# mjq11302010044/TATT

Hardware: AMD Instinct MI355X
Metric: LR images/s (train fwd+bwd+clip+Adam) at 16x64->32x128 (higher is better)
Workload: dtype fp32 (split-bf16 MFMA operands in conv3 / conv3-wgrad / conv9 / tokgemm / gru-wgrad / query-GRU recurrence and dW_hh / TP-layer backward)

## Files before the change

### tatt_amd/csrc/conv9.hip

```cpp
#include "common.h"
#include <mutex>

#define T9_H 8
#define T9_W 32
#define T9_HH (T9_H + 8)
#define T9_WW (T9_W + 8)
#define T9_CK 16

__device__ __forceinline__ void stage_halo_q(const float* __restrict__ x, f32x4 (*Xs)[T9_HH][T9_WW], int n, int h0, int w0,
                                             int H, int W, int C, int c0) {
    for (int i = threadIdx.x; i < T9_HH * T9_WW * 4; i += 256) {
        const int c4 = i & 3, p = i >> 2;
        const int r = p / T9_WW, cc = p - r * T9_WW;
        const int hh = h0 + r - 4, ww = w0 + cc - 4;
        f32x4 v = (f32x4){0.f, 0.f, 0.f, 0.f};
        if (hh >= 0 && hh < H && ww >= 0 && ww < W)
            v = *reinterpret_cast<const f32x4*>(x + (((long)n * H + hh) * W + ww) * C + c0 + 4 * c4);
        Xs[c4][r][cc] = v;
    }
}

__global__ __launch_bounds__(256) void conv9_c64_to_c4_kernel(const float* __restrict__ x, const float* __restrict__ wp,
                                                              const float* __restrict__ bias, float* __restrict__ y,
                                                              int B, int H, int W, int C) {
    __shared__ f32x4 Xs[4][T9_HH][T9_WW];
    const int tiles_w = W / T9_W, tiles_h = H / T9_H;
    int bid = blockIdx.x;
    const int tw = bid % tiles_w; bid /= tiles_w;
    const int th = bid % tiles_h; const int n = bid / tiles_h;
    const int h0 = th * T9_H, w0 = tw * T9_W;
    const int tx = threadIdx.x & 31, ty = threadIdx.x >> 5;
    float a0 = 0.f, a1 = 0.f, a2 = 0.f, a3 = 0.f;
    for (int c0 = 0; c0 < C; c0 += T9_CK) {
        __syncthreads();
        stage_halo_q(x, Xs, n, h0, w0, H, W, C, c0);
        __syncthreads();
        for (int kh = 0; kh < 9; ++kh) {
#pragma unroll
            for (int kw = 0; kw < 9; ++kw) {
                const float* wt = wp + ((long)(kh * 9 + kw) * C + c0) * 4;
#pragma unroll
                for (int c4 = 0; c4 < 4; ++c4) {
                    const f32x4 v = Xs[c4][ty + kh][tx + kw];
#pragma unroll
                    for (int u = 0; u < 4; ++u) {
                        const float* wv = wt + (c4 * 4 + u) * 4;
                        a0 = fmaf(v[u], wv[0], a0); a1 = fmaf(v[u], wv[1], a1);
                        a2 = fmaf(v[u], wv[2], a2); a3 = fmaf(v[u], wv[3], a3);
                    }
                }
            }
        }
    }
    if (bias) { a0 += bias[0]; a1 += bias[1]; a2 += bias[2]; a3 += bias[3]; }
    const long o = (((long)n * H + h0 + ty) * W + w0 + tx) * 4;
    *reinterpret_cast<f32x4*>(y + o) = (f32x4){a0, a1, a2, a3};
}
TATT_API int tatt_conv9_c64_to_c4(const float* x, const float* wpacked, const float* bias, float* y, int B, int H, int W,
                                  int C, hipStream_t st) {
    if (C % T9_CK || H % T9_H || W % T9_W) return 1;
    hipLaunchKernelGGL(conv9_c64_to_c4_kernel, dim3(B * (H / T9_H) * (W / T9_W)), dim3(256), 0, st, x, wpacked, bias, y, B,
                       H, W, C);
    return LAUNCH_CHECK();
}

#define M9_TH 4
#define M9_TW 64
#define M9_PW 96
#define M9_ROWS (M9_TH + 8)
#define M9_HPX (M9_ROWS * 72)
#define M9_HQ 2
#define M9_D 3
#define M9_XS (M9_ROWS * 16 * M9_PW)
__global__ __launch_bounds__(512) void conv9_c64_to_c4_mfma_kernel(const float* __restrict__ x, const float* __restrict__ wt,
                                                                   const float* __restrict__ bias, float* __restrict__ y,
                                                                   int B, int H, int W, int ntiles) {
    __shared__ __attribute__((aligned(16))) float Xs[M9_XS];
    __shared__ __attribute__((aligned(16))) float Red[4 * 64 * 4];
    const int t = threadIdx.x, lane = t & 63, wave = t >> 6;
    const int row = wave & 3, kh = wave >> 2;
    const int tiles_w = W / M9_TW, tiles_h = H / M9_TH;
    const int i = lane & 15, kq = lane >> 4;
    const int g = (i & 8) ? i : (i ^ 4);
    const float* xa = Xs + (row * 16 + 4 * kh + kq) * M9_PW + 4 * g;
    const int wl = (kh * 6 * 64 + lane) * 16;
    const __amdgpu_buffer_rsrc_t wrs = __builtin_amdgcn_make_buffer_rsrc(const_cast<float*>(wt), 0, 9 * 4 * 2 * 6 * 64 * 4 * 4, 0x00020000);
    f32x4 wpre[M9_D + 1][6];
    f32x4 hpre[M9_HQ][4];
    auto filt_load = [&](int p) {
#pragma unroll
        for (int f = 0; f < 6; ++f)
            wpre[p % (M9_D + 1)][f] = __builtin_bit_cast(f32x4, __builtin_amdgcn_raw_buffer_load_b128(
                wrs, wl, (((p % 9) * 4 + p / 9) * 12 + f) * 1024, 0));
    };
    auto halo_load = [&](int tile, int c0, int q) {
        const int tw = tile % tiles_w, th = (tile / tiles_w) % tiles_h, n = tile / (tiles_w * tiles_h);
        const int pp = t + 512 * q;
        const int r = pp / 72, px = pp - r * 72;
        const int hh = th * M9_TH + r - 4, ww = tw * M9_TW + px - 4;
        const bool ok = tile < ntiles && pp < M9_HPX && hh >= 0 && hh < H && ww >= 0 && ww < W;
        const f32x4* src = reinterpret_cast<const f32x4*>(x + (((long)n * H + hh) * W + ww) * 64 + c0);
#pragma unroll
        for (int c4 = 0; c4 < 4; ++c4) hpre[q][c4] = ok ? src[c4] : (f32x4){0.f, 0.f, 0.f, 0.f};
    };
    auto halo_store = [&](int q) {
        const int pp = t + 512 * q;
        if (pp < M9_HPX) {
            const int r = pp / 72, px = pp - r * 72;
            float* d = Xs + r * 16 * M9_PW + px;
#pragma unroll
            for (int c4 = 0; c4 < 4; ++c4)
#pragma unroll
                for (int e = 0; e < 4; ++e) d[(4 * c4 + e) * M9_PW] = hpre[q][c4][e];
        }
    };
#pragma unroll
    for (int q = 0; q < M9_D; ++q) filt_load(q);
#pragma unroll
    for (int q = 0; q < M9_HQ; ++q) halo_load(blockIdx.x, 0, q);
#pragma unroll
    for (int q = 0; q < M9_HQ; ++q) halo_store(q);
    __syncthreads();
    const float bo = bias ? bias[i & 3] : 0.f;
#pragma unroll 1
    for (int tile = blockIdx.x; tile < ntiles; tile += gridDim.x) {
        f32x4 acc4[4];
#pragma unroll
        for (int q = 0; q < 4; ++q) acc4[q] = (f32x4){0.f, 0.f, 0.f, 0.f};
#pragma unroll
        for (int c = 0; c < 4; ++c) {
#pragma unroll
            for (int ky = 0; ky < 9; ++ky) {
                const int p = 9 * c + ky;
                filt_load((p + M9_D) % 36);
                if (ky < M9_HQ) {
                    if (c < 3) halo_load(tile, 16 * (c + 1), ky);
                    else halo_load(tile + gridDim.x, 0, ky);
                }
#pragma unroll
                for (int d = 0; d < 3; ++d) {
                    const f32x4 a0 = *reinterpret_cast<const f32x4*>(xa + (ky * 16 + 0) * M9_PW + 4 * d);
                    const f32x4 a1 = *reinterpret_cast<const f32x4*>(xa + (ky * 16 + 8) * M9_PW + 4 * d);
                    const f32x4 b0 = wpre[p % (M9_D + 1)][d], b1 = wpre[p % (M9_D + 1)][3 + d];
#pragma unroll
                    for (int u = 0; u < 4; ++u) {
                        acc4[u & 1] = __builtin_amdgcn_mfma_f32_16x16x4f32(a0[u], b0[u], acc4[u & 1], 0, 0, 0);
                        acc4[2 + (u & 1)] = __builtin_amdgcn_mfma_f32_16x16x4f32(a1[u], b1[u], acc4[2 + (u & 1)], 0, 0, 0);
                    }
                }
                __builtin_amdgcn_sched_barrier(0);
                if (ky == 8) {
                    f32x4 acc = (acc4[0] + acc4[1]) + (acc4[2] + acc4[3]);
                    __syncthreads();
#pragma unroll
                    for (int q = 0; q < M9_HQ; ++q) halo_store(q);
                    if (c == 3 && kh == 1) *reinterpret_cast<f32x4*>(&Red[(row * 64 + lane) * 4]) = acc;
                    __syncthreads();
                    if (c == 3 && kh == 0) {
                        acc += *reinterpret_cast<const f32x4*>(&Red[(row * 64 + lane) * 4]);
                        const int tw = tile % tiles_w, th = (tile / tiles_w) % tiles_h, n = tile / (tiles_w * tiles_h);
#pragma unroll
                        for (int reg = 0; reg < 4; ++reg) {
                            const int mrow = 4 * kq + reg;
                            const int gg = (mrow & 8) ? mrow : (mrow ^ 4);
                            y[(((long)n * H + th * M9_TH + row) * W + tw * M9_TW + 4 * gg) * 4 + i] = acc[reg] + bo;
                        }
                    }
                }
            }
        }
    }
}
TATT_API int tatt_conv9_c64_to_c4_mfma(const float* x, const float* wt, const float* bias, float* y, int B, int H, int W,
                                       hipStream_t st) {
    if (H % M9_TH || W % M9_TW) return 1;
    const int ntiles = B * (H / M9_TH) * (W / M9_TW);
    hipLaunchKernelGGL(conv9_c64_to_c4_mfma_kernel, dim3(ntiles < 256 ? ntiles : 256), dim3(512), 0, st, x, wt, bias, y, B, H, W,
                       ntiles);
    return LAUNCH_CHECK();
}

#define S9_ROWB (4 * 18 * 32)
#define S9_IMG (M9_ROWS * S9_ROWB)
#define S9_THREADS 768
#define S9_D 5
#define S9_RED (12 * 2 * 64 * 16)
#define S9_LDS (2 * S9_IMG + S9_RED)
typedef __bf16 s9_bf16x8 __attribute__((ext_vector_type(8)));
typedef __bf16 s9_bf16x2 __attribute__((ext_vector_type(2)));
typedef float s9_f32x2 __attribute__((ext_vector_type(2)));
typedef unsigned s9_u32x4 __attribute__((ext_vector_type(4)));
__device__ __forceinline__ void s9_split(f32x4 v, unsigned& h0, unsigned& h1, unsigned& l0, unsigned& l1) {
    const s9_f32x2 a = (s9_f32x2){v[0], v[1]}, b = (s9_f32x2){v[2], v[3]};
    const s9_bf16x2 ha = __builtin_convertvector(a, s9_bf16x2), hb = __builtin_convertvector(b, s9_bf16x2);
    const s9_bf16x2 la = __builtin_convertvector(a - __builtin_convertvector(ha, s9_f32x2), s9_bf16x2);
    const s9_bf16x2 lb = __builtin_convertvector(b - __builtin_convertvector(hb, s9_f32x2), s9_bf16x2);
    h0 = __builtin_bit_cast(unsigned, ha); h1 = __builtin_bit_cast(unsigned, hb);
    l0 = __builtin_bit_cast(unsigned, la); l1 = __builtin_bit_cast(unsigned, lb);
}
__global__ __launch_bounds__(S9_THREADS) void conv9_c64_to_c4_sb_kernel(const float* __restrict__ x, const float* __restrict__ wt,
                                                                        const float* __restrict__ bias, float* __restrict__ y,
                                                                        int B, int H, int W, int ntiles) {
    extern __shared__ __attribute__((aligned(16))) unsigned char s9_lds[];
    unsigned char* const Xs = s9_lds;
    float* const Red = reinterpret_cast<float*>(s9_lds + 2 * S9_IMG);
    const int t = threadIdx.x, lane = t & 63;
    const int wave = __builtin_amdgcn_readfirstlane(t >> 6);
    const int pair = wave % 6, rh = wave / 6;
    const int tiles_w = W / M9_TW, tiles_h = H / M9_TH;
    const int i = lane & 15, kq = lane >> 4;
    const int pair_off = (((2 * pair) & 3) * 18 + (pair >> 1)) * 32;
    int xa[2];
#pragma unroll
    for (int r = 0; r < 2; ++r) xa[r] = (((2 * rh + r) * 4 + (kq >> 1)) * 18 + i) * 32 + (kq & 1) * 16 + pair_off;
    const int wl = (pair * 2 * 64 + lane) * 16;
    const __amdgpu_buffer_rsrc_t wrs = __builtin_amdgcn_make_buffer_rsrc(const_cast<float*>(wt), 0, 9 * 4 * 2 * 6 * 64 * 4 * 4, 0x00020000);
    f32x4 wpre[S9_D + 1][2];
    f32x4 hpre[M9_HQ][4];
    auto filt_load = [&](int p) {
#pragma unroll
        for (int f = 0; f < 2; ++f)
            wpre[p % (S9_D + 1)][f] = __builtin_bit_cast(f32x4, __builtin_amdgcn_raw_buffer_load_b128(
                wrs, wl, (((p % 9) * 4 + p / 9) * 12 + f) * 1024, 0));
    };
    auto halo_load = [&](int tile, int c0, int q) {
        const int tw = tile % tiles_w, th = (tile / tiles_w) % tiles_h, n = tile / (tiles_w * tiles_h);
        const int pp = t + S9_THREADS * q;
        const int r = pp / 72, px = pp - r * 72;
        const int hh = th * M9_TH + r - 4, ww = tw * M9_TW + px - 4;
        const bool ok = tile < ntiles && pp < M9_HPX && hh >= 0 && hh < H && ww >= 0 && ww < W;
        const f32x4* src = reinterpret_cast<const f32x4*>(x + (((long)n * H + hh) * W + ww) * 64 + c0);
#pragma unroll
        for (int c4 = 0; c4 < 4; ++c4) hpre[q][c4] = ok ? src[c4] : (f32x4){0.f, 0.f, 0.f, 0.f};
    };
    auto halo_store = [&](int q) {
        const int pp = t + S9_THREADS * q;
        if (pp < M9_HPX) {
            const int r = pp / 72, px = pp - r * 72;
            unsigned char* d = Xs + ((r * 4 + (px & 3)) * 18 + (px >> 2)) * 32;
            unsigned h[8], l[8];
#pragma unroll
            for (int c4 = 0; c4 < 4; ++c4) s9_split(hpre[q][c4], h[2 * c4], h[2 * c4 + 1], l[2 * c4], l[2 * c4 + 1]);
            *reinterpret_cast<s9_u32x4*>(d) = (s9_u32x4){h[0], h[1], h[2], h[3]};
            *reinterpret_cast<s9_u32x4*>(d + 16) = (s9_u32x4){h[4], h[5], h[6], h[7]};
            *reinterpret_cast<s9_u32x4*>(d + S9_IMG) = (s9_u32x4){l[0], l[1], l[2], l[3]};
            *reinterpret_cast<s9_u32x4*>(d + S9_IMG + 16) = (s9_u32x4){l[4], l[5], l[6], l[7]};
        }
    };
    const int per_img = tiles_w * tiles_h;
    const bool by_xcd = (gridDim.x & 7) == 0 && (B & 7) == 0;
    const int xcd = blockIdx.x & 7, wg_m = blockIdx.x >> 3, wg_M = gridDim.x >> 3;
    auto tile_of = [&](int s) -> int {
        if (!by_xcd) { const long tl = (long)blockIdx.x + (long)s * gridDim.x; return tl < ntiles ? (int)tl : ntiles; }
        const int sq = wg_m + s * wg_M, img = xcd + 8 * (sq / per_img);
        return img < B ? img * per_img + sq % per_img : ntiles;
    };
#pragma unroll
    for (int q = 0; q < S9_D; ++q) filt_load(q);
#pragma unroll
    for (int q = 0; q < M9_HQ; ++q) halo_load(tile_of(0), 0, q);
#pragma unroll
    for (int q = 0; q < M9_HQ; ++q) halo_store(q);
    __syncthreads();
    const float bo = bias ? bias[i & 3] : 0.f;
#pragma unroll 1
    for (int ts = 0;; ++ts) {
        const int tile = tile_of(ts);
        if (tile >= ntiles) break;
        const int tile_next = tile_of(ts + 1);
        f32x4 acc6[2][3];
#pragma unroll
        for (int q = 0; q < 6; ++q) acc6[q / 3][q % 3] = (f32x4){0.f, 0.f, 0.f, 0.f};
#pragma unroll
        for (int c = 0; c < 4; ++c) {
#pragma unroll
            for (int ky = 0; ky < 9; ++ky) {
                const int p = 9 * c + ky;
                filt_load((p + S9_D) % 36);
                if (ky < M9_HQ) {
                    if (c < 3) halo_load(tile, 16 * (c + 1), ky);
                    else halo_load(tile_next, 0, ky);
                }
                const s9_bf16x8 bh = __builtin_bit_cast(s9_bf16x8, wpre[p % (S9_D + 1)][0]);
                const s9_bf16x8 bl = __builtin_bit_cast(s9_bf16x8, wpre[p % (S9_D + 1)][1]);
                s9_bf16x8 ah[2], al[2];
#pragma unroll
                for (int r = 0; r < 2; ++r) {
                    ah[r] = *reinterpret_cast<const s9_bf16x8*>(Xs + xa[r] + ky * S9_ROWB);
                    al[r] = *reinterpret_cast<const s9_bf16x8*>(Xs + xa[r] + ky * S9_ROWB + S9_IMG);
                }
#pragma unroll
                for (int r = 0; r < 2; ++r) {
                    acc6[r][0] = __builtin_amdgcn_mfma_f32_16x16x32_bf16(ah[r], bh, acc6[r][0], 0, 0, 0);
                    acc6[r][1] = __builtin_amdgcn_mfma_f32_16x16x32_bf16(ah[r], bl, acc6[r][1], 0, 0, 0);
                    acc6[r][2] = __builtin_amdgcn_mfma_f32_16x16x32_bf16(al[r], bh, acc6[r][2], 0, 0, 0);
                }
                __builtin_amdgcn_sched_barrier(0);
                if (ky == 8) {
                    __syncthreads();
#pragma unroll
                    for (int q = 0; q < M9_HQ; ++q) halo_store(q);
                    if (c == 3) {
#pragma unroll
                        for (int r = 0; r < 2; ++r)
                            *reinterpret_cast<f32x4*>(&Red[((wave * 2 + r) * 64 + lane) * 4]) = (acc6[r][0] + acc6[r][1]) + acc6[r][2];
                    }
                    __syncthreads();
                    if (c == 3 && pair < 2) {
                        f32x4 acc = (f32x4){0.f, 0.f, 0.f, 0.f};
#pragma unroll
                        for (int pw = 0; pw < 6; ++pw)
                            acc += *reinterpret_cast<const f32x4*>(&Red[(((rh * 6 + pw) * 2 + pair) * 64 + lane) * 4]);
                        const int tw = tile % tiles_w, th = (tile / tiles_w) % tiles_h, n = tile / (tiles_w * tiles_h);
#pragma unroll
                        for (int reg = 0; reg < 4; ++reg)
                            y[(((long)n * H + th * M9_TH + 2 * rh + pair) * W + tw * M9_TW + 4 * (4 * kq + reg)) * 4 + i] = acc[reg] + bo;
                    }
                }
            }
        }
    }
}
TATT_API int tatt_conv9_c64_to_c4_sb(const float* x, const float* wt, const float* bias, float* y, int B, int H, int W,
                                     hipStream_t st) {
    if (H % M9_TH || W % M9_TW) return 1;
    const int ntiles = B * (H / M9_TH) * (W / M9_TW);
    static TattPerDevice attr_once;
    tatt_per_device(attr_once, [&] {
        (void)hipFuncSetAttribute(reinterpret_cast<const void*>(conv9_c64_to_c4_sb_kernel), hipFuncAttributeMaxDynamicSharedMemorySize, S9_LDS);
    });
    hipLaunchKernelGGL(conv9_c64_to_c4_sb_kernel, dim3(ntiles < 256 ? ntiles : 256), dim3(S9_THREADS), S9_LDS, st, x, wt, bias, y, B,
                       H, W, ntiles);
    return LAUNCH_CHECK();
}

#define F9_TH 4
#define F9_TW 64
#define F9_DW (F9_TW + 8)
#define F9_ROWS (F9_TH + 8)
struct F9P { const float* in; const float* wp; const float* bias; float* out; int B, H, W, ntiles, act; };
__global__ __launch_bounds__(512) void conv9_c4_to_c64_kernel(F9P p) {
    __shared__ __attribute__((aligned(16))) float Ds[F9_ROWS * F9_DW * 4];
    const int t = threadIdx.x, lane = t & 63, wave = t >> 6;
    const int nt = wave & 3, half = wave >> 2, li = lane & 15, lk = lane >> 4;
    const int tiles_w = p.W / F9_TW, tiles_h = p.H / F9_TH;
    float wreg[81];
#pragma unroll
    for (int tap = 0; tap < 81; ++tap) wreg[tap] = p.wp[(tap * 4 + lk) * 64 + 16 * nt + li];
    f32x4 bo = (f32x4){0.f, 0.f, 0.f, 0.f};
    if (p.bias) bo = *reinterpret_cast<const f32x4*>(p.bias + 16 * nt + 4 * lk);
    f32x4 dr0, dr1 = (f32x4){0.f, 0.f, 0.f, 0.f};
    auto decode = [&](int tile, int& b, int& h0, int& w0) {
        const int tw = tile % tiles_w; tile /= tiles_w;
        h0 = (tile % tiles_h) * F9_TH; b = tile / tiles_h; w0 = tw * F9_TW;
    };
    auto load1 = [&](int e, int b, int h0, int w0) -> f32x4 {
        const int d = e / F9_DW, q = e - d * F9_DW, row = h0 - 4 + d, px = w0 - 4 + q;
        if (row < 0 || row >= p.H || px < 0 || px >= p.W) return (f32x4){0.f, 0.f, 0.f, 0.f};
        return *reinterpret_cast<const f32x4*>(p.in + (((long)b * p.H + row) * p.W + px) * 4);
    };
    auto load_halo = [&](int tile) {
        int b, h0, w0; decode(tile, b, h0, w0);
        dr0 = load1(t, b, h0, w0);
        if (t < F9_ROWS * F9_DW - 512) dr1 = load1(t + 512, b, h0, w0);
    };
    if ((int)blockIdx.x < p.ntiles) load_halo(blockIdx.x);
    for (int tile = blockIdx.x; tile < p.ntiles; tile += gridDim.x) {
        __syncthreads();
        *reinterpret_cast<f32x4*>(&Ds[4 * t]) = dr0;
        if (t < F9_ROWS * F9_DW - 512) *reinterpret_cast<f32x4*>(&Ds[4 * (t + 512)]) = dr1;
        if (tile + (int)gridDim.x < p.ntiles) load_halo(tile + gridDim.x);
        __syncthreads();
        int b, h0, w0; decode(tile, b, h0, w0);
#pragma unroll 1
        for (int r = 0; r < 2; ++r) {
            const int row = 2 * half + r;
            const float* db = &Ds[(row * F9_DW + li) * 4 + lk];
            f32x4 acc[4];
#pragma unroll
            for (int mg = 0; mg < 4; ++mg) acc[mg] = (f32x4){0.f, 0.f, 0.f, 0.f};
#pragma unroll
            for (int ky = 0; ky < 9; ++ky)
#pragma unroll
                for (int kx = 0; kx < 9; ++kx)
#pragma unroll
                    for (int mg = 0; mg < 4; ++mg)
                        acc[mg] = __builtin_amdgcn_mfma_f32_16x16x4f32(wreg[ky * 9 + kx], db[(ky * F9_DW + kx + 16 * mg) * 4], acc[mg], 0, 0, 0);
            float* o = p.out + (((long)b * p.H + h0 + row) * p.W + w0 + li) * 64 + 16 * nt + 4 * lk;
#pragma unroll
            for (int mg = 0; mg < 4; ++mg) {
                f32x4 v = acc[mg] + bo;
                if (p.act != ACT_NONE) {
#pragma unroll
                    for (int e = 0; e < 4; ++e) v[e] = apply_act(v[e], p.act);
                }
                *reinterpret_cast<f32x4*>(o + (long)16 * mg * 64) = v;
            }
        }
    }
}
TATT_API int tatt_conv9_c4_to_c64(const float* in, const float* wp, const float* bias, float* out, int B, int H, int W, int act,
                                  hipStream_t st) {
    if (H % F9_TH || W % F9_TW) return 1;
    F9P p = {in, wp, bias, out, B, H, W, B * (H / F9_TH) * (W / F9_TW), act};
    const int G = p.ntiles < 256 ? p.ntiles : 256;
    hipLaunchKernelGGL(conv9_c4_to_c64_kernel, dim3(G), dim3(512), 0, st, p);
    return LAUNCH_CHECK();
}

#define G9_IMG (F9_ROWS * F9_DW * 8)
typedef __bf16 g9_bf16x8 __attribute__((ext_vector_type(8)));
typedef unsigned g9_u32x2 __attribute__((ext_vector_type(2)));
__global__ __launch_bounds__(512) void conv9_c4_to_c64_sb_kernel(F9P p) {
    __shared__ __attribute__((aligned(16))) unsigned char Ds[2 * G9_IMG];
    const int t = threadIdx.x, lane = t & 63, wave = t >> 6;
    const int nt = wave & 3, half = wave >> 2, li = lane & 15, lk = lane >> 4;
    const int tiles_w = p.W / F9_TW, tiles_h = p.H / F9_TH;
    g9_bf16x8 wh[11], wl[11];
    int ta[11][2];
#pragma unroll
    for (int m = 0; m < 11; ++m) {
        float v[8];
#pragma unroll
        for (int e = 0; e < 8; ++e) {
            const int tap = 8 * m + 2 * lk + (e >> 2);
            v[e] = tap < 81 ? p.wp[(tap * 4 + (e & 3)) * 64 + 16 * nt + li] : 0.f;
        }
#pragma unroll
        for (int e = 0; e < 8; e += 2) {
            const s9_f32x2 a = (s9_f32x2){v[e], v[e + 1]};
            const s9_bf16x2 h = __builtin_convertvector(a, s9_bf16x2);
            const s9_bf16x2 l = __builtin_convertvector(a - __builtin_convertvector(h, s9_f32x2), s9_bf16x2);
            wh[m][e] = h[0]; wh[m][e + 1] = h[1];
            wl[m][e] = l[0]; wl[m][e + 1] = l[1];
        }
#pragma unroll
        for (int u = 0; u < 2; ++u) {
            const int tap = min(8 * m + 2 * lk + u, 80), ky = tap / 9, kx = tap - 9 * ky;
            ta[m][u] = (((2 * half + ky) * F9_DW) + li + kx) * 8;
        }
    }
    f32x4 bo = (f32x4){0.f, 0.f, 0.f, 0.f};
    if (p.bias) bo = *reinterpret_cast<const f32x4*>(p.bias + 16 * nt + 4 * lk);
    f32x4 dr0, dr1 = (f32x4){0.f, 0.f, 0.f, 0.f};
    auto decode = [&](int tile, int& b, int& h0, int& w0) {
        const int tw = tile % tiles_w; tile /= tiles_w;
        h0 = (tile % tiles_h) * F9_TH; b = tile / tiles_h; w0 = tw * F9_TW;
    };
    auto load1 = [&](int e, int b, int h0, int w0) -> f32x4 {
        const int d = e / F9_DW, q = e - d * F9_DW, row = h0 - 4 + d, px = w0 - 4 + q;
        if (row < 0 || row >= p.H || px < 0 || px >= p.W) return (f32x4){0.f, 0.f, 0.f, 0.f};
        return *reinterpret_cast<const f32x4*>(p.in + (((long)b * p.H + row) * p.W + px) * 4);
    };
    auto load_halo = [&](int tile) {
        int b, h0, w0; decode(tile, b, h0, w0);
        dr0 = load1(t, b, h0, w0);
        if (t < F9_ROWS * F9_DW - 512) dr1 = load1(t + 512, b, h0, w0);
    };
    auto store1 = [&](int e, f32x4 v) {
        unsigned h0, h1, l0, l1;
        s9_split(v, h0, h1, l0, l1);
        *reinterpret_cast<g9_u32x2*>(Ds + e * 8) = (g9_u32x2){h0, h1};
        *reinterpret_cast<g9_u32x2*>(Ds + G9_IMG + e * 8) = (g9_u32x2){l0, l1};
    };
    if ((int)blockIdx.x < p.ntiles) load_halo(blockIdx.x);
    for (int tile = blockIdx.x; tile < p.ntiles; tile += gridDim.x) {
        __syncthreads();
        store1(t, dr0);
        if (t < F9_ROWS * F9_DW - 512) store1(t + 512, dr1);
        if (tile + (int)gridDim.x < p.ntiles) load_halo(tile + gridDim.x);
        __syncthreads();
        int b, h0, w0; decode(tile, b, h0, w0);
#pragma unroll
        for (int r = 0; r < 2; ++r) {
            f32x4 acc[4];
#pragma unroll
            for (int mg = 0; mg < 4; ++mg) acc[mg] = (f32x4){0.f, 0.f, 0.f, 0.f};
#pragma unroll
            for (int m = 0; m < 11; ++m) {
                g9_bf16x8 bh[4], bl[4];
#pragma unroll
                for (int mg = 0; mg < 4; ++mg) {
                    const int off = (r * F9_DW + 16 * mg) * 8;
                    g9_u32x2 q0 = *reinterpret_cast<const g9_u32x2*>(Ds + ta[m][0] + off), q1 = *reinterpret_cast<const g9_u32x2*>(Ds + ta[m][1] + off);
                    g9_u32x2 q2 = *reinterpret_cast<const g9_u32x2*>(Ds + ta[m][0] + off + G9_IMG), q3 = *reinterpret_cast<const g9_u32x2*>(Ds + ta[m][1] + off + G9_IMG);
                    bh[mg] = __builtin_bit_cast(g9_bf16x8, (s9_u32x4){q0[0], q0[1], q1[0], q1[1]});
                    bl[mg] = __builtin_bit_cast(g9_bf16x8, (s9_u32x4){q2[0], q2[1], q3[0], q3[1]});
                }
#pragma unroll
                for (int mg = 0; mg < 4; ++mg) acc[mg] = __builtin_amdgcn_mfma_f32_16x16x32_bf16(wh[m], bh[mg], acc[mg], 0, 0, 0);
#pragma unroll
                for (int mg = 0; mg < 4; ++mg) acc[mg] = __builtin_amdgcn_mfma_f32_16x16x32_bf16(wh[m], bl[mg], acc[mg], 0, 0, 0);
#pragma unroll
                for (int mg = 0; mg < 4; ++mg) acc[mg] = __builtin_amdgcn_mfma_f32_16x16x32_bf16(wl[m], bh[mg], acc[mg], 0, 0, 0);
            }
            const int row = 2 * half + r;
            float* o = p.out + (((long)b * p.H + h0 + row) * p.W + w0 + li) * 64 + 16 * nt + 4 * lk;
#pragma unroll
            for (int mg = 0; mg < 4; ++mg) {
                f32x4 v = acc[mg] + bo;
                if (p.act != ACT_NONE) {
#pragma unroll
                    for (int e = 0; e < 4; ++e) v[e] = apply_act(v[e], p.act);
                }
                *reinterpret_cast<f32x4*>(o + (long)16 * mg * 64) = v;
            }
        }
    }
}
TATT_API int tatt_conv9_c4_to_c64_sb(const float* in, const float* wp, const float* bias, float* out, int B, int H, int W, int act,
                                     hipStream_t st) {
    if (H % F9_TH || W % F9_TW) return 1;
    F9P p = {in, wp, bias, out, B, H, W, B * (H / F9_TH) * (W / F9_TW), act};
    const int G = p.ntiles < 256 ? p.ntiles : 256;
    hipLaunchKernelGGL(conv9_c4_to_c64_sb_kernel, dim3(G), dim3(512), 0, st, p);
    return LAUNCH_CHECK();
}

#define W9_R 4
#define W9_P 64
#define W9_XP 80
#define W9_DW (W9_P + 8)
#define W9_DROWS (W9_R + 8)
#define W9_NT 21
#define W9_N (W9_NT * 16)
struct W9P { const float* x; const float* dy; float* part; int B, H, W, ntiles, flip; };
__global__ __launch_bounds__(768) void conv9_c64_c4_wgrad_mfma_kernel(W9P p) {
    __shared__ __attribute__((aligned(16))) float Xs[2][W9_P * W9_XP];
    __shared__ __attribute__((aligned(16))) float Ds[(W9_DROWS + 1) * W9_DW * 4];
    const int t = threadIdx.x, lane = t & 63, wave = t >> 6;
    const int mt = wave & 3, ng = wave >> 2, li = lane & 15, lk = lane >> 4;
    const int tiles_w = p.W / W9_P, tiles_h = p.H / W9_R;
    int bbase[7], bstep[7];
#pragma unroll
    for (int j = 0; j < 7; ++j) {
        const int n = 16 * (7 * ng + j) + li, tap = n >> 2, co = n & 3;
        if (tap < 81) {
            const int ky = tap / 9, kx = tap - 9 * ky;
            bbase[j] = p.flip ? (ky * W9_DW + lk + kx) * 4 + co : ((8 - ky) * W9_DW + lk + 8 - kx) * 4 + co;
            bstep[j] = W9_DW * 4;
        } else { bbase[j] = W9_DROWS * W9_DW * 4; bstep[j] = 0; }
    }
    for (int e = t; e < W9_DW * 4; e += 768) Ds[W9_DROWS * W9_DW * 4 + e] = 0.f;
    f32x4 acc[7];
#pragma unroll
    for (int j = 0; j < 7; ++j) acc[j] = (f32x4){0.f, 0.f, 0.f, 0.f};
    const int my_tiles = p.ntiles > (int)blockIdx.x ? (p.ntiles - 1 - (int)blockIdx.x) / (int)gridDim.x + 1 : 0;
    const int nsteps = my_tiles * W9_R;
    f32x4 xr0, xr1 = (f32x4){0.f, 0.f, 0.f, 0.f}, dr0, dr1 = (f32x4){0.f, 0.f, 0.f, 0.f};
    auto tile_of = [&](int s, int& b, int& r0, int& p0) {
        int tile = blockIdx.x + (s / W9_R) * gridDim.x;
        const int tw = tile % tiles_w; tile /= tiles_w;
        r0 = (tile % tiles_h) * W9_R; b = tile / tiles_h; p0 = tw * W9_P;
    };
    auto load_x = [&](int s) {
        int b, r0, p0; tile_of(s, b, r0, p0);
        const float* src = p.x + (((long)b * p.H + r0 + s % W9_R) * p.W + p0) * 64;
        xr0 = *reinterpret_cast<const f32x4*>(src + 4 * t);
        if (t < 256) xr1 = *reinterpret_cast<const f32x4*>(src + 4 * (t + 768));
    };
    auto store_x = [&](int buf) {
        *reinterpret_cast<f32x4*>(&Xs[buf][(t >> 4) * W9_XP + 4 * (t & 15)]) = xr0;
        if (t < 256) *reinterpret_cast<f32x4*>(&Xs[buf][((t + 768) >> 4) * W9_XP + 4 * (t & 15)]) = xr1;
    };
    auto load_d1 = [&](int e, int b, int r0, int p0) -> f32x4 {
        const int d = e / W9_DW, q = e - d * W9_DW, row = r0 - 4 + d, px = p0 - 4 + q;
        if (row < 0 || row >= p.H || px < 0 || px >= p.W) return (f32x4){0.f, 0.f, 0.f, 0.f};
        return *reinterpret_cast<const f32x4*>(p.dy + (((long)b * p.H + row) * p.W + px) * 4);
    };
    auto load_d = [&](int s) {
        int b, r0, p0; tile_of(s, b, r0, p0);
        dr0 = load_d1(t, b, r0, p0);
        if (t < W9_DROWS * W9_DW - 768) dr1 = load_d1(t + 768, b, r0, p0);
    };
    auto store_d = [&]() {
        *reinterpret_cast<f32x4*>(&Ds[4 * t]) = dr0;
        if (t < W9_DROWS * W9_DW - 768) *reinterpret_cast<f32x4*>(&Ds[4 * (t + 768)]) = dr1;
    };
    if (nsteps > 0) { load_x(0); load_d(0); }
    for (int s = 0; s < nsteps; ++s) {
        const int rr = s % W9_R, buf = s & 1;
        if (rr == 0) __syncthreads();
        store_x(buf);
        if (rr == 0) store_d();
        if (s + 1 < nsteps) { load_x(s + 1); if (rr == W9_R - 1) load_d(s + 1); }
        __syncthreads();
        const float* xa = &Xs[buf][lk * W9_XP + 16 * mt + li];
        const float* db[7];
#pragma unroll
        for (int j = 0; j < 7; ++j) db[j] = &Ds[bbase[j] + rr * bstep[j]];
#pragma unroll 4
        for (int ks = 0; ks < W9_P / 4; ++ks) {
            const float a = xa[ks * 4 * W9_XP];
#pragma unroll
            for (int j = 0; j < 7; ++j) acc[j] = __builtin_amdgcn_mfma_f32_16x16x4f32(a, db[j][ks * 16], acc[j], 0, 0, 0);
        }
    }
    float* P = p.part + (long)blockIdx.x * 64 * W9_N;
#pragma unroll
    for (int j = 0; j < 7; ++j)
#pragma unroll
        for (int e = 0; e < 4; ++e) P[(long)(16 * mt + 4 * lk + e) * W9_N + 16 * (7 * ng + j) + li] = acc[j][e];
}
#define W9S_XP 82
#define W9S_NFRAG 50
#define W9S_XS (2 * W9_P * W9S_XP)
#define W9S_DS ((W9_DROWS + 1) * W9_DW * 4)
#define W9S_LDS ((W9S_XS + W9S_DS) * 4 + W9S_NFRAG * 2 * 64 * 16)
__device__ __forceinline__ void w9s_frag(const float* __restrict__ col, int stride, g9_bf16x8& hi, g9_bf16x8& lo) {
    float v[8];
#pragma unroll
    for (int e = 0; e < 8; ++e) v[e] = col[e * stride];
#pragma unroll
    for (int e = 0; e < 8; e += 2) {
        const s9_f32x2 a = (s9_f32x2){v[e], v[e + 1]};
        const s9_bf16x2 h = __builtin_convertvector(a, s9_bf16x2);
        const s9_bf16x2 l = __builtin_convertvector(a - __builtin_convertvector(h, s9_f32x2), s9_bf16x2);
        hi[e] = h[0]; hi[e + 1] = h[1];
        lo[e] = l[0]; lo[e + 1] = l[1];
    }
}
__global__ __launch_bounds__(768) void conv9_c64_c4_wgrad_sb_kernel(W9P p) {
    extern __shared__ __attribute__((aligned(16))) float w9s_lds[];
    float* const Xs = w9s_lds;
    float* const Ds = w9s_lds + W9S_XS;
    f32x4* const Fr = reinterpret_cast<f32x4*>(w9s_lds + W9S_XS + W9S_DS);
    const int t = threadIdx.x, lane = t & 63;
    const int wave = __builtin_amdgcn_readfirstlane(t >> 6);
    const int mt = wave & 3, ng = wave >> 2, li = lane & 15, lk = lane >> 4;
    const int tiles_w = p.W / W9_P, tiles_h = p.H / W9_R;
    int gb[5], gs[5], gr[5];
#pragma unroll
    for (int q = 0; q < 5; ++q) {
        const int f = wave + 12 * q;
        if (f < 8) {
            gb[q] = ((f & 1) * 32 + 8 * lk) * W9S_XP + 16 * (f >> 1) + li; gs[q] = W9S_XP; gr[q] = 0;
        } else {
            const int ntile = (f - 8) >> 1, ks = (f - 8) & 1;
            const int n = 16 * ntile + li, tap = n >> 2, co = n & 3;
            if (tap < 81 && f < W9S_NFRAG) {
                const int ky = tap / 9, kx = tap - 9 * ky;
                gb[q] = W9S_XS + (p.flip ? (ky * W9_DW + 8 * lk + kx) * 4 + co : ((8 - ky) * W9_DW + 8 * lk + 8 - kx) * 4 + co) + ks * 128;
                gr[q] = W9_DW * 4;
            } else { gb[q] = W9S_XS + W9_DROWS * W9_DW * 4; gr[q] = 0; }
            gs[q] = 4;
        }
    }
    for (int e = t; e < W9_DW * 4; e += 768) Ds[W9_DROWS * W9_DW * 4 + e] = 0.f;
    f32x4 acc[7];
#pragma unroll
    for (int j = 0; j < 7; ++j) acc[j] = (f32x4){0.f, 0.f, 0.f, 0.f};
    const int my_tiles = p.ntiles > (int)blockIdx.x ? (p.ntiles - 1 - (int)blockIdx.x) / (int)gridDim.x + 1 : 0;
    const int nsteps = my_tiles * W9_R;
    f32x4 xr0, xr1 = (f32x4){0.f, 0.f, 0.f, 0.f}, dr0, dr1 = (f32x4){0.f, 0.f, 0.f, 0.f};
    auto tile_of = [&](int s, int& b, int& r0, int& p0) {
        int tile = blockIdx.x + (s / W9_R) * gridDim.x;
        const int tw = tile % tiles_w; tile /= tiles_w;
        r0 = (tile % tiles_h) * W9_R; b = tile / tiles_h; p0 = tw * W9_P;
    };
    auto load_x = [&](int s) {
        int b, r0, p0; tile_of(s, b, r0, p0);
        const float* src = p.x + (((long)b * p.H + r0 + s % W9_R) * p.W + p0) * 64;
        xr0 = *reinterpret_cast<const f32x4*>(src + 4 * t);
        if (t < 256) xr1 = *reinterpret_cast<const f32x4*>(src + 4 * (t + 768));
    };
    auto store_x = [&](int buf) {
        float* d0 = Xs + buf * W9_P * W9S_XP + (t >> 4) * W9S_XP + 4 * (t & 15);
        *reinterpret_cast<float2*>(d0) = make_float2(xr0[0], xr0[1]);
        *reinterpret_cast<float2*>(d0 + 2) = make_float2(xr0[2], xr0[3]);
        if (t < 256) {
            float* d1 = Xs + buf * W9_P * W9S_XP + ((t + 768) >> 4) * W9S_XP + 4 * (t & 15);
            *reinterpret_cast<float2*>(d1) = make_float2(xr1[0], xr1[1]);
            *reinterpret_cast<float2*>(d1 + 2) = make_float2(xr1[2], xr1[3]);
        }
    };
    auto load_d1 = [&](int e, int b, int r0, int p0) -> f32x4 {
        const int d = e / W9_DW, q = e - d * W9_DW, row = r0 - 4 + d, px = p0 - 4 + q;
        if (row < 0 || row >= p.H || px < 0 || px >= p.W) return (f32x4){0.f, 0.f, 0.f, 0.f};
        return *reinterpret_cast<const f32x4*>(p.dy + (((long)b * p.H + row) * p.W + px) * 4);
    };
    auto load_d = [&](int s) {
        int b, r0, p0; tile_of(s, b, r0, p0);
        dr0 = load_d1(t, b, r0, p0);
        if (t < W9_DROWS * W9_DW - 768) dr1 = load_d1(t + 768, b, r0, p0);
    };
    auto store_d = [&]() {
        *reinterpret_cast<f32x4*>(&Ds[4 * t]) = dr0;
        if (t < W9_DROWS * W9_DW - 768) *reinterpret_cast<f32x4*>(&Ds[4 * (t + 768)]) = dr1;
    };
    if (nsteps > 0) { load_x(0); load_d(0); }
    for (int s = 0; s < nsteps; ++s) {
        const int rr = s % W9_R, buf = s & 1;
        store_x(buf);
        if (rr == 0) store_d();
        if (s + 1 < nsteps) { load_x(s + 1); if (rr == W9_R - 1) load_d(s + 1); }
        __syncthreads();
#pragma unroll
        for (int q = 0; q < 5; ++q) {
            const int f = wave + 12 * q;
            if (f < W9S_NFRAG) {
                g9_bf16x8 hi, lo;
                w9s_frag(w9s_lds + gb[q] + (f < 8 ? buf * W9_P * W9S_XP : rr * gr[q]), gs[q], hi, lo);
                Fr[(f * 2 + 0) * 64 + lane] = __builtin_bit_cast(f32x4, hi);
                Fr[(f * 2 + 1) * 64 + lane] = __builtin_bit_cast(f32x4, lo);
            }
        }
        __syncthreads();
#pragma unroll
        for (int ks = 0; ks < 2; ++ks) {
            const g9_bf16x8 ah = __builtin_bit_cast(g9_bf16x8, Fr[((2 * mt + ks) * 2 + 0) * 64 + lane]);
            const g9_bf16x8 al = __builtin_bit_cast(g9_bf16x8, Fr[((2 * mt + ks) * 2 + 1) * 64 + lane]);
            g9_bf16x8 bh[7], bl[7];
#pragma unroll
            for (int j = 0; j < 7; ++j) {
                const int f = 8 + 2 * (7 * ng + j) + ks;
                bh[j] = __builtin_bit_cast(g9_bf16x8, Fr[(f * 2 + 0) * 64 + lane]);
                bl[j] = __builtin_bit_cast(g9_bf16x8, Fr[(f * 2 + 1) * 64 + lane]);
            }
#pragma unroll
            for (int j = 0; j < 7; ++j) acc[j] = __builtin_amdgcn_mfma_f32_16x16x32_bf16(ah, bh[j], acc[j], 0, 0, 0);
#pragma unroll
            for (int j = 0; j < 7; ++j) acc[j] = __builtin_amdgcn_mfma_f32_16x16x32_bf16(ah, bl[j], acc[j], 0, 0, 0);
#pragma unroll
            for (int j = 0; j < 7; ++j) acc[j] = __builtin_amdgcn_mfma_f32_16x16x32_bf16(al, bh[j], acc[j], 0, 0, 0);
        }
    }
    float* P = p.part + (long)blockIdx.x * 64 * W9_N;
#pragma unroll
    for (int j = 0; j < 7; ++j)
#pragma unroll
        for (int e = 0; e < 4; ++e) P[(long)(16 * mt + 4 * lk + e) * W9_N + 16 * (7 * ng + j) + li] = acc[j][e];
}
__global__ __launch_bounds__(1024) void conv9_wgrad_reduce_kernel(const float* __restrict__ part, float* __restrict__ dw, int G,
                                                                  int swap) {
    __shared__ float sh[16][64];
    const int tx = threadIdx.x & 63, ty = threadIdx.x >> 6;
    const int idx = blockIdx.x * 64 + tx;
    const int ci = idx / 324, n = idx - ci * 324;
    const float* src = part + (long)ci * W9_N + n;
    float s0 = 0.f, s1 = 0.f, s2 = 0.f, s3 = 0.f;
    int g = ty;
    for (; g + 48 < G; g += 64) {
        s0 += src[(long)g * 64 * W9_N]; s1 += src[(long)(g + 16) * 64 * W9_N];
        s2 += src[(long)(g + 32) * 64 * W9_N]; s3 += src[(long)(g + 48) * 64 * W9_N];
    }
    for (; g < G; g += 16) s0 += src[(long)g * 64 * W9_N];
    sh[ty][tx] = (s0 + s1) + (s2 + s3);
    __syncthreads();
    if (ty == 0) {
        float s = 0.f;
#pragma unroll
        for (int l = 0; l < 16; ++l) s += sh[l][tx];
        dw[(swap ? (long)ci * 4 + (n & 3) : (long)(n & 3) * 64 + ci) * 81 + (n >> 2)] = s;
    }
}
static int conv9_wgrad_launch(const float* x64, const float* t4, float* dw, float* part, int B, int H, int W, int flip,
                              hipStream_t st, bool sb = false) {
    if (H % W9_R || W % W9_P) return 1;
    W9P p = {x64, t4, part, B, H, W, B * (H / W9_R) * (W / W9_P), flip};
    const int G = p.ntiles < 256 ? p.ntiles : 256;
    if (sb) {
        static TattPerDevice attr_once;
        tatt_per_device(attr_once, [&] {
            (void)hipFuncSetAttribute(reinterpret_cast<const void*>(conv9_c64_c4_wgrad_sb_kernel), hipFuncAttributeMaxDynamicSharedMemorySize, W9S_LDS);
        });
        hipLaunchKernelGGL(conv9_c64_c4_wgrad_sb_kernel, dim3(G), dim3(768), W9S_LDS, st, p);
    }
    else hipLaunchKernelGGL(conv9_c64_c4_wgrad_mfma_kernel, dim3(G), dim3(768), 0, st, p);
    hipLaunchKernelGGL(conv9_wgrad_reduce_kernel, dim3(64 * 324 / 64), dim3(1024), 0, st, part, dw, G, flip);
    return LAUNCH_CHECK();
}
TATT_API int tatt_conv9_c64_c4_wgrad(const float* x, const float* dy, float* dw, float* part, int B, int H, int W,
                                     hipStream_t st) {
    return conv9_wgrad_launch(x, dy, dw, part, B, H, W, 0, st);
}
TATT_API int tatt_conv9_c4_c64_wgrad(const float* x, const float* dy, float* dw, float* part, int B, int H, int W,
                                     hipStream_t st) {
    return conv9_wgrad_launch(dy, x, dw, part, B, H, W, 1, st);
}
TATT_API int tatt_conv9_c64_c4_wgrad_sb(const float* x, const float* dy, float* dw, float* part, int B, int H, int W,
                                        hipStream_t st) {
    return conv9_wgrad_launch(x, dy, dw, part, B, H, W, 0, st, true);
}
TATT_API int tatt_conv9_c4_c64_wgrad_sb(const float* x, const float* dy, float* dw, float* part, int B, int H, int W,
                                        hipStream_t st) {
    return conv9_wgrad_launch(dy, x, dw, part, B, H, W, 1, st, true);
}
```

Before: 11800.

## Warp-specialize conv9 split-bf16 kernel with dedicated halo loader waves and two-tile batching

Splits the conv9 split-bf16 kernel's workgroup into six compute waves and two loader waves. The loader waves stream halo channel slices into a double-buffered LDS staging area. Compute waves now each own a channel-pair slice across all four output rows, reusing each loaded LDS row across several ky taps. Filter rows for a whole channel group are held in registers and refilled during compute, and two tiles are processed per iteration. The aim is to take global loads and the bf16 split off the MFMA critical path and raise LDS-row reuse, at the cost of more registers, a larger LDS footprint and barrier-coupled producer/consumer scheduling.

```diff
diff --git a/tatt_amd/csrc/conv9.hip b/tatt_amd/csrc/conv9.hip
--- a/tatt_amd/csrc/conv9.hip
+++ b/tatt_amd/csrc/conv9.hip
@@ -1,5 +1,6 @@
 #include "common.h"
 #include <mutex>
+#include <type_traits>
 
 #define T9_H 8
 #define T9_W 32
@@ -182,10 +183,15 @@
 
 #define S9_ROWB (4 * 18 * 32)
 #define S9_IMG (M9_ROWS * S9_ROWB)
-#define S9_THREADS 768
-#define S9_D 5
-#define S9_RED (12 * 2 * 64 * 16)
-#define S9_LDS (2 * S9_IMG + S9_RED)
+#define S9_BUF (2 * S9_IMG)
+#define S9_CW 6
+#define S9_LT 128
+#define S9_THREADS (64 * S9_CW + S9_LT)
+#define S9_T 2
+#define S9_RED (S9_CW * 4 * 64 * 16)
+#define S9_LDS (2 * S9_BUF + S9_T * S9_RED)
+#define S9_HU (2 * M9_HPX)
+#define S9_HK ((S9_HU + S9_LT - 1) / S9_LT)
 typedef __bf16 s9_bf16x8 __attribute__((ext_vector_type(8)));
 typedef __bf16 s9_bf16x2 __attribute__((ext_vector_type(2)));
 typedef float s9_f32x2 __attribute__((ext_vector_type(2)));
@@ -203,49 +209,26 @@
                                                                         int B, int H, int W, int ntiles) {
     extern __shared__ __attribute__((aligned(16))) unsigned char s9_lds[];
     unsigned char* const Xs = s9_lds;
-    float* const Red = reinterpret_cast<float*>(s9_lds + 2 * S9_IMG);
+    float* const Red = reinterpret_cast<float*>(s9_lds + 2 * S9_BUF);
     const int t = threadIdx.x, lane = t & 63;
     const int wave = __builtin_amdgcn_readfirstlane(t >> 6);
-    const int pair = wave % 6, rh = wave / 6;
+    const bool loader = wave >= S9_CW;
+    const int pair = loader ? 0 : wave;
     const int tiles_w = W / M9_TW, tiles_h = H / M9_TH;
     const int i = lane & 15, kq = lane >> 4;
-    const int pair_off = (((2 * pair) & 3) * 18 + (pair >> 1)) * 32;
-    int xa[2];
-#pragma unroll
-    for (int r = 0; r < 2; ++r) xa[r] = (((2 * rh + r) * 4 + (kq >> 1)) * 18 + i) * 32 + (kq & 1) * 16 + pair_off;
+    const int xa = ((kq >> 1) * 18 + i) * 32 + (kq & 1) * 16 + (((2 * pair) & 3) * 18 + (pair >> 1)) * 32;
     const int wl = (pair * 2 * 64 + lane) * 16;
     const __amdgpu_buffer_rsrc_t wrs = __builtin_amdgcn_make_buffer_rsrc(const_cast<float*>(wt), 0, 9 * 4 * 2 * 6 * 64 * 4 * 4, 0x00020000);
-    f32x4 wpre[S9_D + 1][2];
-    f32x4 hpre[M9_HQ][4];
-    auto filt_load = [&](int p) {
+    f32x4 wst[9][2];
+    auto filt_load_row = [&](int c, int ky) {
 #pragma unroll
         for (int f = 0; f < 2; ++f)
-            wpre[p % (S9_D + 1)][f] = __builtin_bit_cast(f32x4, __builtin_amdgcn_raw_buffer_load_b128(
-                wrs, wl, (((p % 9) * 4 + p / 9) * 12 + f) * 1024, 0));
-    };
-    auto halo_load = [&](int tile, int c0, int q) {
-        const int tw = tile % tiles_w, th = (tile / tiles_w) % tiles_h, n = tile / (tiles_w * tiles_h);
-        const int pp = t + S9_THREADS * q;
-        const int r = pp / 72, px = pp - r * 72;
-        const int hh = th * M9_TH + r - 4, ww = tw * M9_TW + px - 4;
-        const bool ok = tile < ntiles && pp < M9_HPX && hh >= 0 && hh < H && ww >= 0 && ww < W;
-        const f32x4* src = reinterpret_cast<const f32x4*>(x + (((long)n * H + hh) * W + ww) * 64 + c0);
-#pragma unroll
-        for (int c4 = 0; c4 < 4; ++c4) hpre[q][c4] = ok ? src[c4] : (f32x4){0.f, 0.f, 0.f, 0.f};
-    };
-    auto halo_store = [&](int q) {
-        const int pp = t + S9_THREADS * q;
-        if (pp < M9_HPX) {
-            const int r = pp / 72, px = pp - r * 72;
-            unsigned char* d = Xs + ((r * 4 + (px & 3)) * 18 + (px >> 2)) * 32;
-            unsigned h[8], l[8];
-#pragma unroll
-            for (int c4 = 0; c4 < 4; ++c4) s9_split(hpre[q][c4], h[2 * c4], h[2 * c4 + 1], l[2 * c4], l[2 * c4 + 1]);
-            *reinterpret_cast<s9_u32x4*>(d) = (s9_u32x4){h[0], h[1], h[2], h[3]};
-            *reinterpret_cast<s9_u32x4*>(d + 16) = (s9_u32x4){h[4], h[5], h[6], h[7]};
-            *reinterpret_cast<s9_u32x4*>(d + S9_IMG) = (s9_u32x4){l[0], l[1], l[2], l[3]};
-            *reinterpret_cast<s9_u32x4*>(d + S9_IMG + 16) = (s9_u32x4){l[4], l[5], l[6], l[7]};
-        }
+            wst[ky][f] = __builtin_bit_cast(f32x4, __builtin_amdgcn_raw_buffer_load_b128(
+                wrs, wl, c * (12 * 1024) + (ky * 48 + f) * 1024, 0));
+    };
+    auto filt_load = [&](int c) {
+#pragma unroll
+        for (int ky = 0; ky < 9; ++ky) filt_load_row(c, ky);
     };
     const int per_img = tiles_w * tiles_h;
     const bool by_xcd = (gridDim.x & 7) == 0 && (B & 7) == 0;
@@ -255,67 +238,138 @@
         const int sq = wg_m + s * wg_M, img = xcd + 8 * (sq / per_img);
         return img < B ? img * per_img + sq % per_img : ntiles;
     };
-#pragma unroll
-    for (int q = 0; q < S9_D; ++q) filt_load(q);
-#pragma unroll
-    for (int q = 0; q < M9_HQ; ++q) halo_load(tile_of(0), 0, q);
-#pragma unroll
-    for (int q = 0; q < M9_HQ; ++q) halo_store(q);
+    if (loader) {
+        const int lt = t - 64 * S9_CW;
+        f32x4 hpre[S9_HK][2];
+        int ts = 0, it = 0, tile_a = tile_of(0), tile_b = tile_of(1);
+        auto advance = [&]() {
+            const bool two = tile_b < ntiles;
+            if (++it == (two ? 8 : 4)) { it = 0; ts += S9_T; tile_a = tile_of(ts); tile_b = tile_of(ts + 1); }
+        };
+        auto halo_load = [&]() {
+            const bool two = tile_b < ntiles;
+            const int tile = __builtin_amdgcn_readfirstlane((two && (it & 1)) ? tile_b : tile_a);
+            const int c0 = __builtin_amdgcn_readfirstlane(16 * (two ? it >> 1 : it));
+            const int tw = tile % tiles_w, th = (tile / tiles_w) % tiles_h, n = tile / (tiles_w * tiles_h);
+            const float* const xt = x + (((long)n * H + th * M9_TH - 4) * W + tw * M9_TW - 4) * 64 + c0;
+            const __amdgpu_buffer_rsrc_t xrs = __builtin_amdgcn_make_buffer_rsrc(const_cast<float*>(xt), 0, 0x7fffffff, 0x00020000);
+#pragma unroll
+            for (int k = 0; k < S9_HK; ++k) {
+                const int u = lt + S9_LT * k;
+                const int pp = u >> 1, r = pp / 72, px = pp - r * 72;
+                const int hh = th * M9_TH + r - 4, ww = tw * M9_TW + px - 4;
+                const bool ok = u < S9_HU && (unsigned)hh < (unsigned)H && (unsigned)ww < (unsigned)W;
+                const int off = ok ? ((r * W + px) * 64 + 8 * (u & 1)) * 4 : (int)0x80000000;
+#pragma unroll
+                for (int c4 = 0; c4 < 2; ++c4)
+                    hpre[k][c4] = __builtin_bit_cast(f32x4, __builtin_amdgcn_raw_buffer_load_b128(xrs, off + 16 * c4, 0, 0));
+            }
+        };
+        auto halo_store = [&](int buf) {
+#pragma unroll
+            for (int k = 0; k < S9_HK; ++k) {
+                const int u = lt + S9_LT * k;
+                if (u < S9_HU) {
+                    const int pp = u >> 1, r = pp / 72, px = pp - r * 72;
+                    unsigned char* d = Xs + buf * S9_BUF + ((r * 4 + (px & 3)) * 18 + (px >> 2)) * 32 + 16 * (u & 1);
+                    unsigned h[4], l[4];
+#pragma unroll
+                    for (int c4 = 0; c4 < 2; ++c4) s9_split(hpre[k][c4], h[2 * c4], h[2 * c4 + 1], l[2 * c4], l[2 * c4 + 1]);
+                    *reinterpret_cast<s9_u32x4*>(d) = (s9_u32x4){h[0], h[1], h[2], h[3]};
+                    *reinterpret_cast<s9_u32x4*>(d + S9_IMG) = (s9_u32x4){l[0], l[1], l[2], l[3]};
+                }
+            }
+        };
+        halo_load();
+        halo_store(0);
+        advance();
+        bool v1 = tile_a < ntiles;
+        if (v1) halo_load();
+        __syncthreads();
+#pragma unroll 1
+        for (int k = 0;; ++k) {
+            if (v1) halo_store((k + 1) & 1);
+            bool v2 = false;
+            if (v1) { advance(); v2 = tile_a < ntiles; }
+            if (v2) halo_load();
+            __syncthreads();
+            if (!v1) break;
+            v1 = v2;
+        }
+        return;
+    }
+    filt_load(0);
     __syncthreads();
     const float bo = bias ? bias[i & 3] : 0.f;
 #pragma unroll 1
-    for (int ts = 0;; ++ts) {
-        const int tile = tile_of(ts);
-        if (tile >= ntiles) break;
-        const int tile_next = tile_of(ts + 1);
-        f32x4 acc6[2][3];
-#pragma unroll
-        for (int q = 0; q < 6; ++q) acc6[q / 3][q % 3] = (f32x4){0.f, 0.f, 0.f, 0.f};
-#pragma unroll
-        for (int c = 0; c < 4; ++c) {
-#pragma unroll
-            for (int ky = 0; ky < 9; ++ky) {
-                const int p = 9 * c + ky;
-                filt_load((p + S9_D) % 36);
-                if (ky < M9_HQ) {
-                    if (c < 3) halo_load(tile, 16 * (c + 1), ky);
-                    else halo_load(tile_next, 0, ky);
-                }
-                const s9_bf16x8 bh = __builtin_bit_cast(s9_bf16x8, wpre[p % (S9_D + 1)][0]);
-                const s9_bf16x8 bl = __builtin_bit_cast(s9_bf16x8, wpre[p % (S9_D + 1)][1]);
-                s9_bf16x8 ah[2], al[2];
-#pragma unroll
-                for (int r = 0; r < 2; ++r) {
-                    ah[r] = *reinterpret_cast<const s9_bf16x8*>(Xs + xa[r] + ky * S9_ROWB);
-                    al[r] = *reinterpret_cast<const s9_bf16x8*>(Xs + xa[r] + ky * S9_ROWB + S9_IMG);
-                }
-#pragma unroll
-                for (int r = 0; r < 2; ++r) {
-                    acc6[r][0] = __builtin_amdgcn_mfma_f32_16x16x32_bf16(ah[r], bh, acc6[r][0], 0, 0, 0);
-                    acc6[r][1] = __builtin_amdgcn_mfma_f32_16x16x32_bf16(ah[r], bl, acc6[r][1], 0, 0, 0);
-                    acc6[r][2] = __builtin_amdgcn_mfma_f32_16x16x32_bf16(al[r], bh, acc6[r][2], 0, 0, 0);
-                }
+    for (int ts = 0;; ts += S9_T) {
+        const int tile_a = tile_of(ts);
+        if (tile_a >= ntiles) break;
+        const int tile_b = tile_of(ts + 1);
+        const bool two = tile_b < ntiles;
+        f32x4 acc[S9_T][4][3];
+#pragma unroll
+        for (int q = 0; q < 12 * S9_T; ++q) acc[q / 12][(q / 3) & 3][q % 3] = (f32x4){0.f, 0.f, 0.f, 0.f};
+        auto item = [&](auto B_, auto REFILL_, int c, int cur) __attribute__((always_inline)) {
+            constexpr int b = decltype(B_)::value;
+            constexpr bool refill = decltype(REFILL_)::value;
+            const unsigned char* const Xc = Xs + cur * S9_BUF + xa;
+            s9_bf16x8 ah = *reinterpret_cast<const s9_bf16x8*>(Xc);
+            s9_bf16x8 al = *reinterpret_cast<const s9_bf16x8*>(Xc + S9_IMG);
+#pragma unroll
+            for (int rho = 0; rho < M9_ROWS; ++rho) {
+                const s9_bf16x8 ah0 = ah, al0 = al;
+                if (rho + 1 < M9_ROWS) {
+                    ah = *reinterpret_cast<const s9_bf16x8*>(Xc + (rho + 1) * S9_ROWB);
+                    al = *reinterpret_cast<const s9_bf16x8*>(Xc + (rho + 1) * S9_ROWB + S9_IMG);
+                }
+#pragma unroll
+                for (int r = 0; r < 4; ++r) {
+                    const int ky = rho - r;
+                    if (ky >= 0 && ky < 9) {
+                        const s9_bf16x8 bh = __builtin_bit_cast(s9_bf16x8, wst[ky][0]);
+                        const s9_bf16x8 bl = __builtin_bit_cast(s9_bf16x8, wst[ky][1]);
+                        acc[b][r][0] = __builtin_amdgcn_mfma_f32_16x16x32_bf16(ah0, bh, acc[b][r][0], 0, 0, 0);
+                        acc[b][r][1] = __builtin_amdgcn_mfma_f32_16x16x32_bf16(ah0, bl, acc[b][r][1], 0, 0, 0);
+                        acc[b][r][2] = __builtin_amdgcn_mfma_f32_16x16x32_bf16(al0, bh, acc[b][r][2], 0, 0, 0);
+                    }
+                }
+                if (refill && rho >= 3) filt_load_row((c + 1) & 3, rho - 3);
                 __builtin_amdgcn_sched_barrier(0);
-                if (ky == 8) {
-                    __syncthreads();
-#pragma unroll
-                    for (int q = 0; q < M9_HQ; ++q) halo_store(q);
-                    if (c == 3) {
-#pragma unroll
-                        for (int r = 0; r < 2; ++r)
-                            *reinterpret_cast<f32x4*>(&Red[((wave * 2 + r) * 64 + lane) * 4]) = (acc6[r][0] + acc6[r][1]) + acc6[r][2];
-                    }
-                    __syncthreads();
-                    if (c == 3 && pair < 2) {
-                        f32x4 acc = (f32x4){0.f, 0.f, 0.f, 0.f};
-#pragma unroll
-                        for (int pw = 0; pw < 6; ++pw)
-                            acc += *reinterpret_cast<const f32x4*>(&Red[(((rh * 6 + pw) * 2 + pair) * 64 + lane) * 4]);
-                        const int tw = tile % tiles_w, th = (tile / tiles_w) % tiles_h, n = tile / (tiles_w * tiles_h);
-#pragma unroll
-                        for (int reg = 0; reg < 4; ++reg)
-                            y[(((long)n * H + th * M9_TH + 2 * rh + pair) * W + tw * M9_TW + 4 * (4 * kq + reg)) * 4 + i] = acc[reg] + bo;
-                    }
+            }
+            if (c == 3) {
+#pragma unroll
+                for (int r = 0; r < 4; ++r)
+                    *reinterpret_cast<f32x4*>(&Red[(((b * S9_CW + pair) * 4 + r) * 64 + lane) * 4]) =
+                        (acc[b][r][0] + acc[b][r][1]) + acc[b][r][2];
+            }
+            __syncthreads();
+        };
+        using s9_i0 = std::integral_constant<int, 0>;
+        using s9_i1 = std::integral_constant<int, 1>;
+        if (two) {
+#pragma unroll 1
+            for (int c = 0; c < 4; ++c) {
+                item(s9_i0{}, std::false_type{}, c, 0);
+                item(s9_i1{}, std::true_type{}, c, 1);
+            }
+        } else {
+#pragma unroll 1
+            for (int c = 0; c < 4; ++c) item(s9_i0{}, std::true_type{}, c, c & 1);
+        }
+        if (wave < 4) {
+#pragma unroll
+            for (int b = 0; b < S9_T; ++b) {
+                if (b == 0 || two) {
+                    const int tile = b ? tile_b : tile_a;
+                    f32x4 o = (f32x4){0.f, 0.f, 0.f, 0.f};
+#pragma unroll
+                    for (int pw = 0; pw < S9_CW; ++pw)
+                        o += *reinterpret_cast<const f32x4*>(&Red[(((b * S9_CW + pw) * 4 + wave) * 64 + lane) * 4]);
+                    const int tw = tile % tiles_w, th = (tile / tiles_w) % tiles_h, n = tile / (tiles_w * tiles_h);
+#pragma unroll
+                    for (int reg = 0; reg < 4; ++reg)
+                        y[(((long)n * H + th * M9_TH + wave) * W + tw * M9_TW + 4 * (4 * kq + reg)) * 4 + i] = o[reg] + bo;
                 }
             }
         }
```

After: 11850, median of 6. No clear change (+0.5%).
